# acerbilab/vbmc

Measured on AMD Instinct MI355X. Metric: ELBO+grad evals/sec (Ns=1e4, K=50, D=10, N=400), higher is better.
Workload: dtype f64; 1 GPU; BASELINE configs[2]: D=10 N=400 K=50 Ns=10000/component S=20, R=64 restarts batched per GPU per step, value+gradient, beta=0, no variance; restarts_per_gpu=64, parallelism=one GPU

## Files before the change

### vbmc_amd/csrc/abi_elbo.hip

```cpp
#include <algorithm>
#include <cmath>
#include <mutex>

#include "elbo_kernels.h"
#include "var_kernels.h"
#include "gp_kernels.h"
#include <cstdlib>

extern "C" int vbmc_abi_version(void) { return VBMC_ABI_VERSION; }

static vbmc_status ctx_create_impl(int device, void* stream, vbmc_ctx** out, bool with_aux) {
  if (!out) return VBMC_ERR_INVALID;
  *out = nullptr;
  {
    static std::once_flag hq_once;
    std::call_once(hq_once, [] {
      const char* hq = getenv("VBMC_HW_QUEUES");
      if (!(hq && !strcmp(hq, "0"))) (void)setenv("GPU_MAX_HW_QUEUES", hq && atoi(hq) > 0 ? hq : "8", 0);
    });
  }
  int ndev = 0;
  if (hipGetDeviceCount(&ndev) != hipSuccess || ndev <= 0) return VBMC_ERR_NO_DEVICE;
  if (device < 0 || device >= ndev) return VBMC_ERR_NO_DEVICE;
  hipDeviceProp_t prop;
// ... 362 lines not shown
  if (qs < 1 || qs > 9) return false;
  return fns[qs - 1](kt, grad ? 1 : 0, hv, g.x, g.y, g.z, (void*)st, &ea) == 0;
}
static int entropy_mfma_occupancy(int qs, int kt, int hv, bool grad, const EntArgs& ea) {
  typedef int (*fn_t)(int, int, int, const EntArgs*);
  static const fn_t fns[9] = {vbmc_occupancy_ent_mfma_qs1, vbmc_occupancy_ent_mfma_qs2, vbmc_occupancy_ent_mfma_qs3,
                              vbmc_occupancy_ent_mfma_qs4, vbmc_occupancy_ent_mfma_qs5, vbmc_occupancy_ent_mfma_qs6,
                              vbmc_occupancy_ent_mfma_qs7, vbmc_occupancy_ent_mfma_qs8, vbmc_occupancy_ent_mfma_qs9};
  if (qs < 1 || qs > 9) return -1;
  struct Key { int qs, kt, hv, grad, co, sparse, ldsk; };
  static std::vector<std::pair<Key, int>> cache;
  static std::mutex mu;
  std::lock_guard<std::mutex> lock(mu);
  const Key k{qs, kt, hv, grad ? 1 : 0, ea.lj.rows > 0 ? 1 : 0, ea.cutoff > 0.0 ? 1 : 0, ea.K * (ea.D + ENTP_EXTRA)};
  for (const auto& c : cache)
    if (c.first.qs == k.qs && c.first.kt == k.kt && c.first.hv == k.hv && c.first.grad == k.grad && c.first.co == k.co &&
        c.first.sparse == k.sparse && c.first.ldsk == k.ldsk) return c.second;
  const int nb = fns[qs - 1](kt, grad ? 1 : 0, hv, &ea);
  cache.push_back({k, nb});
  return nb;
}
static bool mfma_entropy_fits(int D, int K, double cutoff, int* qs_out, int* kt_out, int* hv_out) {
  const int qs = (D + 2 + 3) / 4;
  int hv = K <= 64 ? ent_hv_small(qs, K) : (K <= 128 ? ent_hv_mid(qs, K) : (K <= 256 ? 4 : 8));
  if (K > 64 && K <= 128)
    if (const char* f = getenv("VBMC_ENT_HV")) { const int v = atoi(f); if (v == 2 || v == 4) hv = v; }
  if (K > 32 && K <= 64)
    if (const char* f = getenv("VBMC_ENT_HV")) { const int v = atoi(f); if (v == 1 || v == 2) hv = v; }
  int kt = (((K + hv - 1) / hv) + 15) / 16;
  static const bool tail_on = [] { const char* e = getenv("VBMC_ENT_TAIL"); return !(e && !strcmp(e, "0")); }();
  {
    const int Kh = (K + hv - 1) / hv;
    static const int tail_max = [] { const char* e = getenv("VBMC_ENT_TAIL"); return e ? atoi(e) : 2; }();
    const int tl = (Kh % 16 + 3) / 4;
    const int ktf = Kh / 16, rem = Kh % 16;
    const bool tail8_ok = ktf == 1 || (hv == 1 && ktf == 2 && (qs >= 5 || rem <= 6)) || (hv == 1 && ktf == 3 && qs <= 4) ||
                          (hv > 1 && ktf == 2) || (hv > 1 && ktf == 3 && qs >= 5);
    if (tail_on && hv != 8 && Kh > 16 && tl >= 1 && tl <= tail_max && (tl == 1 || (tl == 2 && tail8_ok)) && !(cutoff > 0.0) && !(hv > 1 && ktf < 2)) {
      kt = ktf;
      hv += 16 * tl;
    }
  }
  *qs_out = qs; *kt_out = kt; *hv_out = hv;
  return qs >= 1 && qs <= 9 && K >= 1 && K <= 512 && kt >= 1 && kt <= 4 && !(hv == 2 && kt < 2) && !(hv == 4 && kt < 2) && !(hv == 8 && kt < 3) && !(hv > 16 && kt > 3);
}

#define COPY_KERNEL_MAX_BYTES ((size_t)4 << 20)
__global__ void k_copy_f64(size_t n, const double* __restrict__ src, double* __restrict__ dst) {
  VB_SMALL_PRIO();
  for (size_t i = (size_t)blockIdx.x * blockDim.x + threadIdx.x; i < n; i += (size_t)gridDim.x * blockDim.x) dst[i] = src[i];
}
__global__ void k_copy_rows_f64(int rows, size_t stride, size_t width, const double* __restrict__ src, double* __restrict__ dst) {
  VB_SMALL_PRIO();
  for (int r = blockIdx.y; r < rows; r += gridDim.y)
    for (size_t i = (size_t)blockIdx.x * blockDim.x + threadIdx.x; i < width; i += (size_t)gridDim.x * blockDim.x)
      dst[(size_t)r * stride + i] = src[(size_t)r * stride + i];
}
__global__ void k_pack_sepk(int R, int S, int K, int LJS, int diag_only, const double* __restrict__ lj, const double* __restrict__ J,
                            double* __restrict__ hI, double* __restrict__ hJ) {
  const size_t nI = (size_t)R * S * K, nJ = J ? (size_t)R * S * K * K : 0;
  for (size_t i = (size_t)blockIdx.x * blockDim.x + threadIdx.x; i < nI + nJ; i += (size_t)gridDim.x * blockDim.x) {
    if (i < nI) {
      const int s = (int)(i % S), k = (int)((i / S) % K), r = (int)(i / ((size_t)S * K));
      hI[i] = lj[(((size_t)r * S + s) * K + k) * LJS];
    } else {
      const size_t q = i - nI;
      const int s = (int)(q % S), j = (int)((q / S) % K), k = (int)((q / ((size_t)S * K)) % K), r = (int)(q / ((size_t)S * K * K));
      hJ[q] = (diag_only && j != k) ? 0.0 : J[(((size_t)r * S + s) * K + k) * K + j];
    }
  }
}

static bool copy_by_kernel(size_t bytes) { return bytes <= COPY_KERNEL_MAX_BYTES; }
// ... 1145 lines not shown
  return VBMC_OK;
}

static int limit_T_vargrad() {
  int T = 1;
  while (VAR_FINAL_LDS(1, 1, T + 1) <= 160 * 1024) ++T;
  return T;
}
extern "C" vbmc_status vbmc_get_limits(vbmc_limits* out) {
  if (!out || out->struct_size != sizeof(vbmc_limits)) return VBMC_ERR_INVALID;
  out->max_D = VBMC_LIM_D;
  out->max_K = VBMC_LIM_K;
  out->max_N = trsm_max_n();
  out->max_Na = VBMC_LIM_NA;
  out->max_T_vargrad = limit_T_vargrad();
  out->delta_ok = 1;
  out->meanfun_mask = VBMC_LIM_MEANFUN_MASK;
  return VBMC_OK;
}

extern "C" int vbmc_entropy_plan(int D, int K, int* qs, int* kt, int* hv, int* tail) {
  if (lane_entropy_fits(D, K, 0.0)) {
    if (qs) *qs = 2 * ((D + 1) / 2);
    if (kt) *kt = 2 * ((K + 1) / 2);
    if (hv) *hv = ENT_LANE_WAVES_HOST;
    if (tail) *tail = 0;
    return 2;
  }
  int q = 0, k = 0, h = 0;
  const bool ok = mfma_entropy_fits(D, K, 0.0, &q, &k, &h);
  if (qs) *qs = q;
  if (kt) *kt = k;
  if (hv) *hv = h & 15;
  if (tail) *tail = h >> 4;
  return ok ? 1 : 0;
}

#ifdef VBMC_INSTRUMENT
extern "C" int vbmc_dbg_fin_read(unsigned long long* out) {
  return (int)hipMemcpyFromSymbol(out, HIP_SYMBOL(g_fin_dbg), 64 * sizeof(unsigned long long), 0, hipMemcpyDeviceToHost);
}
#endif

__global__ void k_test_exp(int n, int variant, const double* __restrict__ x, double* __restrict__ y) {
  __shared__ double tab[VB_EXP_TAB_N];
  for (int t = threadIdx.x; t < VB_EXP_TAB_N; t += blockDim.x) tab[t] = c_exp2_tab[t];
  __syncthreads();
  int i = blockIdx.x * blockDim.x + threadIdx.x;
  if (i < n) y[i] = variant == 2 ? vb_exp_tab<1>(x[i], tab) : (variant ? vb_exp_tab<0>(x[i], tab) : vb_exp(x[i]));
}

#include "exp2_tab1k.h"
__global__ void k_test_exp1k(int n, int variant, const double* __restrict__ x, double* __restrict__ y) {
  __shared__ double tab[VB_EXP_TAB1K_N];
  for (int t = threadIdx.x; t < VB_EXP_TAB1K_N; t += blockDim.x) tab[t] = c_exp2_tab1k[t];
  __syncthreads();
  int i = blockIdx.x * blockDim.x + threadIdx.x;
  if (i < n) {
    double ys;
    asm volatile("v_mul_f64 %0, %1, %2" : "=v"(ys) : "v"(x[i]), "v"(VB_EXP_TAB1K_SCALE));
    const bool quad = variant == 3 ? VB_EXP_TAB1K_QUAD : variant == 5;
    y[i] = quad ? vb_exp_tab1k<true>(ys, tab) : vb_exp_tab1k<false>(ys, tab);
  }
}

extern "C" vbmc_status vbmc_test_exp(vbmc_ctx* ctx, int n, int variant, const double* x, double* y) {
  if (!ctx || n <= 0 || !x || !y) return VBMC_ERR_INVALID;
// ... 28 lines not shown
```

### vbmc_amd/csrc/ent_mfma_inst.hip

```cpp
#include "entropy_mfma.h"

#ifndef QS_VALUE
#error "compile with -DQS_VALUE=<1..9>"
#endif
#define CAT2(a, b) a##b
#define CAT(a, b) CAT2(a, b)

template <int KT, int HV, int TL = 0>
static int launch_kt(int mode, int grad, dim3 grid, hipStream_t st, const EntArgs& ea) {
  constexpr int NPV_ = (4 * QS_VALUE + 15) / 16;
  size_t lds = (size_t)ea.K * (ea.D + ENTP_EXTRA) * sizeof(double);
  size_t after = (size_t)VB_EXP_TAB1K_N * sizeof(double);
  if (HV > 1) after += (size_t)(VBMC_ENT_EO(HV) ? 1 : 2) * HV * NPV_ * 4 * WAVE * sizeof(double);
  if (after > lds) lds = after;
  const void* fn = nullptr;
  if constexpr (HV == 1 && QS_VALUE <= 8) {
    if (ea.lj.rows > 0) fn = (const void*)k_entropy_mfma<QS_VALUE, KT, true, false, 1, TL, true>;
  }
  const bool walk = ea.walk_tpw > 0;
  if (walk && !(HV == 1 && QS_VALUE <= 4 && KT <= 3 && grad && !fn && !ea.eps && !(ea.cutoff > 0.0))) return mode != 0 ? -1 : 1;
  if constexpr (HV == 1 && QS_VALUE <= 4 && KT <= 3) {
    if (!fn && grad && !ea.eps && !(ea.cutoff > 0.0))
      fn = walk ? (const void*)k_entropy_mfma<QS_VALUE, KT, true, false, 1, TL, false, false, true> : (const void*)k_entropy_mfma<QS_VALUE, KT, true, false, 1, TL, false, false>;
  }
// ... 1 lines not shown
    if (ea.cutoff > 0.0 && HV == 1 && !TL) {
      if constexpr (HV == 1 && TL == 0)
        fn = grad ? (const void*)k_entropy_mfma<QS_VALUE, KT, true, true, 1> : (const void*)k_entropy_mfma<QS_VALUE, KT, false, true, 1>;
    } else {
      fn = grad ? (const void*)k_entropy_mfma<QS_VALUE, KT, true, false, HV, TL> : (const void*)k_entropy_mfma<QS_VALUE, KT, false, false, HV, TL>;
    }
  }
  if (lds > 64 * 1024) (void)hipFuncSetAttribute(fn, hipFuncAttributeMaxDynamicSharedMemorySize, (int)lds);
  const int threads = (ea.cutoff > 0.0 && HV == 1 && !TL) ? WAVE : WAVE * HV;
  if (mode == 1) {
    int nb = 0;
    if (hipOccupancyMaxActiveBlocksPerMultiprocessor(&nb, fn, threads, lds) != hipSuccess) { (void)hipGetLastError(); return 0; }
    return nb;
  }
  EntArgs arg = ea;
  void* args[] = {(void*)&arg};
  (void)hipLaunchKernel(fn, grid, dim3(threads), args, lds, st);
  return 0;
}

static int dispatch(int mode, int kt, int grad, int hv, dim3 grid, hipStream_t st, const EntArgs* ea) {
  switch (kt + 16 * hv) {
    case 16 + 1: return launch_kt<1, 1>(mode, grad, grid, st, *ea);
    case 16 + 2: return launch_kt<2, 1>(mode, grad, grid, st, *ea);
    case 16 + 3: return launch_kt<3, 1>(mode, grad, grid, st, *ea);
    case 16 + 4: return launch_kt<4, 1>(mode, grad, grid, st, *ea);
    case 272 + 1: return launch_kt<1, 1, 1>(mode, grad, grid, st, *ea);
    case 272 + 2: return launch_kt<2, 1, 1>(mode, grad, grid, st, *ea);
    case 272 + 3: return launch_kt<3, 1, 1>(mode, grad, grid, st, *ea);
    case 288 + 2: return launch_kt<2, 2, 1>(mode, grad, grid, st, *ea);
    case 288 + 3: return launch_kt<3, 2, 1>(mode, grad, grid, st, *ea);
    case 320 + 2: return launch_kt<2, 4, 1>(mode, grad, grid, st, *ea);
    case 320 + 3: return launch_kt<3, 4, 1>(mode, grad, grid, st, *ea);
    case 528 + 1: return launch_kt<1, 1, 2>(mode, grad, grid, st, *ea);
    case 528 + 2: return launch_kt<2, 1, 2>(mode, grad, grid, st, *ea);
    case 528 + 3: return launch_kt<3, 1, 2>(mode, grad, grid, st, *ea);
    case 544 + 2: return launch_kt<2, 2, 2>(mode, grad, grid, st, *ea);
    case 544 + 3: return launch_kt<3, 2, 2>(mode, grad, grid, st, *ea);
    case 576 + 2: return launch_kt<2, 4, 2>(mode, grad, grid, st, *ea);
    case 576 + 3: return launch_kt<3, 4, 2>(mode, grad, grid, st, *ea);
    case 32 + 2: return launch_kt<2, 2>(mode, grad, grid, st, *ea);
    case 32 + 3: return launch_kt<3, 2>(mode, grad, grid, st, *ea);
    case 32 + 4: return launch_kt<4, 2>(mode, grad, grid, st, *ea);
    case 64 + 2: return launch_kt<2, 4>(mode, grad, grid, st, *ea);
    case 64 + 3: return launch_kt<3, 4>(mode, grad, grid, st, *ea);
    case 64 + 4: return launch_kt<4, 4>(mode, grad, grid, st, *ea);
    case 128 + 3: return launch_kt<3, 8>(mode, grad, grid, st, *ea);
    case 128 + 4: return launch_kt<4, 8>(mode, grad, grid, st, *ea);
    default: return mode != 0 ? -1 : 1;
  }
}

extern "C" int CAT(vbmc_launch_ent_mfma_qs, QS_VALUE)(int kt, int grad, int hv, unsigned gx, unsigned gy, unsigned gz, void* stream,
                                                      const EntArgs* ea) {
  return dispatch(0, kt, grad, hv, dim3(gx, gy, gz), (hipStream_t)stream, ea);
}

extern "C" int CAT(vbmc_occupancy_ent_mfma_qs, QS_VALUE)(int kt, int grad, int hv, const EntArgs* ea) {
  return dispatch(1, kt, grad, hv, dim3(1, 1, 1), nullptr, ea);
}

#ifdef VBMC_INSTRUMENT
extern "C" int CAT(vbmc_dbg_ent_read_qs, QS_VALUE)(unsigned long long* out, size_t n) {
  return (int)hipMemcpyFromSymbol(out, HIP_SYMBOL(g_ent_dbg), n * sizeof(unsigned long long), 0, hipMemcpyDeviceToHost);
}
#endif
// ... 1 lines not shown
```

### vbmc_amd/csrc/entropy_mfma.h

```cpp
#pragma once
#include <type_traits>

#include "device_math.h"
#include "elbo_types.h"
#include "exp2_tab1k.h"
#include "logjoint_body.h"

typedef double mf4 __attribute__((ext_vector_type(4)));
struct EntTileAny { static constexpr bool rt = false, val = true; };
struct EntTileFull { static constexpr bool rt = false, val = false; };
struct EntTilePartial { static constexpr bool rt = false, val = true; };
#define VBMC_ENT_SPLIT(KT_, QS_, TL_, HV_) ((HV_) == 1)

#ifdef VBMC_INSTRUMENT
#define VBMC_DBG_WAVES 32768
__device__ unsigned long long g_ent_dbg[6 * VBMC_DBG_WAVES];
#endif

#define VBMC_STAG_FOR(KT_, QS_, TL_) ((KT_) == 1 || (KT_) == 4 || ((KT_) == 2 && (QS_) >= 6) || ((KT_) == 3 && (QS_) <= ((TL_) ? 5 : 8)))



constexpr bool ent_c2_for(int KT, int QS, int TL, int HV) {
  if (HV == 1) {
// ... 7 lines not shown
    if (KT == 3) return !((TL == 1 && (QS == 5 || QS == 6)) || (TL == 2 && QS == 6));
    return true;
  }
  if (KT == 2) return !((TL == 1 && QS >= 6) || (TL == 2 && QS >= 5));
  if (KT == 3) return !(TL == 1 && QS == 7);
  return QS != 5;
}
constexpr bool ent_gp2_for(int KT, int QS, int TL, int HV) { return !(HV == 1 && KT == 1 && TL == 0 && QS <= 3); }

template <int HV>
__device__ __forceinline__ void ent_sync() {
  __builtin_amdgcn_fence(__ATOMIC_RELEASE, "wavefront");
  __builtin_amdgcn_wave_barrier();
  __builtin_amdgcn_fence(__ATOMIC_ACQUIRE, "wavefront");
}
template <int HV>
__device__ __forceinline__ void ent_sync_wg() {
  if (HV == 1) ent_sync<1>();
  else __syncthreads();
}

template <int QS, int KT, bool GRAD, bool SPARSE, int HV = 1, int TL = 0, bool CO = false, bool EM = true, bool WALK = false>
#define VBMC_ENT_EO(HV_) true
#define VBMC_ENT_ONE_WAVE(KT_, QS_, TL_, HV_) \
  (((HV_) == 1 && (KT_) == 4 && (QS_) >= 5) || ((HV_) == 1 && (KT_) == 3 && (QS_) >= 8) || ((HV_) == 4 && (KT_) == 4 && (QS_) >= 6) || \
   ((HV_) == 4 && (KT_) == 3 && (QS_) >= 9))
#define VBMC_ENT_WAVES(KT_, QS_, TL_, HV_) \
  (VBMC_ENT_ONE_WAVE(KT_, QS_, TL_, HV_) ? 1 : ((((KT_) <= 2 && (QS_) <= 4) && !((KT_) == 2 && (TL_) == 2 && (HV_) == 1)) ? 3 : 2))
__device__ __forceinline__ void ent_mfma_segment(const EntArgs& a, const int c, const int j, const int r, const int t0, const int t1,
                                                 const int pdone, const int ptot) {
  static_assert(!CO || (HV == 1 && QS <= 8 && !SPARSE), "the log-joint role exists for single-wave dense kernels at D <= 30");
  static_assert(!WALK || (HV == 1 && !CO), "the walk exists for single-wave workgroups without the log-joint role");
  static_assert(KT <= 4 && (HV == 1 || HV == 2 || HV == 4 || HV == 8), "larger mixtures are split over the waves of a workgroup (HV = 2, 4; round 5: 8, K <= 512)");
  static_assert(TL == 0 || ((TL == 1 || TL == 2) && !SPARSE), "the component tail (one or two values per lane) exists for the dense kernels only");
  constexpr int TLN = TL > 0 ? TL : 1;
  constexpr bool SP = SPARSE;
  constexpr int DP = 4 * QS;
  constexpr int NPV = (4 * QS + 15) / 16;
  constexpr int QL = QS;
  __shared__ double Et[16 * DP];
  constexpr bool GP2 = GRAD && ent_gp2_for(KT, QS, TL, HV);
  __shared__ double RQ_all[HV][GP2 ? 32 : 16];
  __shared__ double BND_all[HV][SPARSE ? KT * 16 * 3 : 1];
  constexpr int YXN = NPV * 4 * WAVE;
  constexpr bool EO = VBMC_ENT_EO(HV);
  constexpr bool YXSB = HV > 1 && EO;
  constexpr bool US = EO;
  constexpr bool VBL = GRAD && HV == 1 && (KT >= 3 || NPV >= 2);
  __shared__ double VBS_all[HV][VBL ? KT * 4 * NPV * WAVE : 1];
  constexpr bool C2 = EO && !SPARSE && ent_c2_for(KT, QS, TL, HV);
#define ENT_CI(kt_, rr_) (16 * (kt_) + 4 * (rr_) + lg)
  __shared__ __attribute__((aligned(16))) double SCP_all[HV][C2 ? KT * 16 * 2 : 2];
  __shared__ double BTL_all[HV][TL ? 4 * TL * DP : 1];
  constexpr bool NML = HV > 1 && EO;
  __shared__ double NMS_all[HV][NML ? KT * 4 * WAVE : 1];
#ifdef VBMC_INSTRUMENT
  const unsigned long long wckE = wall_clock64();
#endif
  int tid_ = threadIdx.x;
  if (WALK) asm volatile("" : "+v"(tid_));
  const int tid = tid_, wv = tid >> 6, hv = HV == 1 ? 0 : wv, lane = tid & 63;
  const int li = lane & 15, lg = lane >> 4;
  int D_ = a.D, K_ = a.K;
  const double *entp_ = a.entp, *vpd_ = a.vpd;
  double* part_ = a.part;
  if (WALK) asm volatile("" : "+s"(D_), "+s"(K_), "+s"(entp_), "+s"(vpd_), "+s"(part_));
  const int D = D_, K = K_;
  double* RQ = RQ_all[wv];
  double* NMS = NMS_all[wv];
  double* BND = BND_all[hv];
  double* VBS = VBS_all[hv];
  double* BTL = BTL_all[hv];
  double* SCP = SCP_all[hv];
  const int Kh = (K + HV - 1) / HV;
  const int kbase = hv * Kh;
  const int Kw = min(K, kbase + Kh) - kbase;
  const int PSg = D + ENTP_EXTRA;
  extern __shared__ double PB[];
  double* const TAB = PB;
  double* const YX = PB + VB_EXP_TAB1K_N;
  constexpr int NTH0 = WAVE * HV;
  constexpr int NTB0 = (VB_EXP_TAB1K_N + NTH0 - 1) / NTH0;
  double tt[NTB0];
#pragma unroll
  for (int u = 0; u < NTB0; ++u) tt[u] = c_exp2_tab1k[min(tid + u * NTH0, VB_EXP_TAB1K_N - 1)];
  const double sigj = vpd_[(size_t)r * VpLayout{D, K}.stride() + VpLayout{D, K}.sigma() + j];
// ... 61 lines not shown
        else if (cc == D) v = h + hj_neg;
        else if (cc == D + 1) v = fma(h, m2, pk[D + 1]) - cKj;
        else v = 0.0;
        SA[kt][q] = ESC * v;
      }
    }
    SC[kt] = ESC * (!kv ? (lg == 1 ? -1.0e6 : 0.0)
                        : (lg == 0 ? h + hj_neg : (lg == 1 ? fma(h, m2, pk[D + 1]) - cKj : 0.0)));
    if (C2 && lg < 2) SCP[(16 * kt + li) * 2 + lg] = 2.0 * SC[kt];
#pragma unroll
    for (int rr = 0; rr < 4; ++rr) {
      const int k2 = ENT_CI(kt, rr);
      const bool kv2 = k2 < Kw;
      const double* p2 = gp + (size_t)(kv2 ? kbase + k2 : 0) * PSg;
      if (GRAD) {
#pragma unroll
        for (int pv = 0; pv < NPV; ++pv) {
          const int col = 16 * pv + li;
          double v = 0.0;
          if (kv2) {
            if (col == 0) v = p2[D + 2];
            else if (col == 1) v = p2[D + 3];
            else if (col < 2 + D) v = p2[D + 3] * (p2[col - 2] - pj[col - 2]);
          }
          if (VBL) VBS[((kt * 4 + rr) * NPV + pv) * WAVE + lane] = v;
          else VB[VBL ? 0 : kt][rr][pv] = v;
        }
      } else {
        WF[kt][rr] = kv2 ? p2[D + 2] : 0.0;
      }
    }
  }

  double tC0[TLN], tC1[TLN], VBt[TLN][NPV], WFt[TLN], Wt[TLN];
#pragma unroll
  for (int u = 0; u < TLN; ++u) {
    tC0[u] = 0.0; tC1[u] = 0.0; WFt[u] = 0.0; Wt[u] = 0.0;
#pragma unroll
    for (int pv = 0; pv < NPV; ++pv) VBt[u][pv] = 0.0;
  }
  if (TL) {
#pragma unroll
    for (int u = 0; u < TLN; ++u) {
      const int tq = 4 * u + lg;
      const int kq = 16 * KT + tq;
      const bool kvq = kq < Kw;
      const double* pq = gp + (size_t)(kvq ? kbase + kq : 0) * PSg;
      const double h = pq[D];
      double m2 = 0.0;
      for (int d = 0; d < D; ++d) { double t = pq[d] - pj[d]; m2 = fma(t, t, m2); }
      tC0[u] = kvq ? ESC * (h + hj_neg) : 0.0;
      tC1[u] = ESC * (kvq ? fma(h, m2, pq[D + 1]) - cKj : -1.0e6);
      for (int d = li; d < DP; d += 16) BTL[tq * DP + d] = (kvq && d < D) ? ESC * (-2.0 * h * (pq[d] - pj[d])) : 0.0;
      if (GRAD) {
#pragma unroll
        for (int pv = 0; pv < NPV; ++pv) {
          const int col = 16 * pv + li;
          double v = 0.0;
          if (kvq) {
            if (col == 0) v = pq[D + 2];
            else if (col == 1) v = pq[D + 3];
            else if (col < 2 + D) v = pq[D + 3] * (pq[col - 2] - pj[col - 2]);
          }
          VBt[u][pv] = v;
        }
      } else {
        WFt[u] = kvq ? pq[D + 2] : 0.0;
      }
    }
  }

  __syncthreads();
  {
#pragma unroll
    for (int u = 0; u < NTB0; ++u) if (VB_EXP_TAB1K_N % NTH0 == 0 || tid + u * NTH0 < VB_EXP_TAB1K_N) TAB[tid + u * NTH0] = tt[u];
  }
  __syncthreads();

#define SAV(kt_, q_) SA[kt_][q_]
  constexpr int VBR = (VBL && NPV == 1 && HV == 1 && KT == 3 && !CO) ? ((EM && QS <= 4) ? (TL == 2 ? 4 : 10) : 12) : 0;
  double VBreg[VBR > 0 ? VBR : 1];
#pragma unroll
  for (int u = 0; u < VBR; ++u) VBreg[u] = VBS[u * WAVE + lane];
#define VBV(kt_, rr_, pv_) (VBL ? (((kt_) * 4 + (rr_)) * NPV + (pv_) < VBR ? VBreg[(((kt_) * 4 + (rr_)) * NPV + (pv_)) < VBR ? (((kt_) * 4 + (rr_)) * NPV + (pv_)) : 0] : VBS[(((kt_) * 4 + (rr_)) * NPV + (pv_)) * WAVE + lane]) : VB[VBL ? 0 : (kt_)][rr_][pv_])
  double accH = 0.0, accG[NPV], accLG[NPV];
  double pm = 1.0;
  int pe = 0, pcnt = 0;
  double Wacc[KT][4];
#pragma unroll
  for (int pv = 0; pv < NPV; ++pv) { accG[pv] = 0.0; accLG[pv] = 0.0; }
#pragma unroll
  for (int kt = 0; kt < KT; ++kt)
#pragma unroll
    for (int rr = 0; rr < 4; ++rr) Wacc[kt][rr] = 0.0;

#ifdef VBMC_INSTRUMENT
  const unsigned long long wck0 = wall_clock64();
#endif
  const int ntile = (a.Mh + 15) >> 4;
  const double sfm0 = lg == 0 ? 1.0 : 0.0, sfm1 = lg == 1 ? 1.0 : 0.0;
  const int emask = (4 * (QS - 1) + lg < D) ? -1 : 0;
  const int emask2 = (QS >= 2 && 4 * (QS - 2) + lg < D) ? -1 : 0;
  const double* epsr = a.eps ? a.eps + (size_t)r * a.eps_stride_r + (size_t)j * a.Mh * D : nullptr;
  constexpr bool EPF = EM && HV == 1 && QS <= 4 && KT <= 3 && !SPARSE;
  double epre[EPF ? QS : 1];
  auto eps_fetch = [&](const int tile) {
#pragma unroll
    for (int u = 0; u < (EPF ? QS : 0); ++u) {
      const int idx = lane + u * WAVE, i = idx / DP, d = idx - i * DP;
      double v = 0.0;
      if (tile < t1 && d < D && tile * 16 + i < a.Mh) v = epsr[(size_t)(tile * 16 + i) * D + d];
      epre[u] = v;
    }
  };
  if (EPF && epsr) eps_fetch(t0);
  if (!epsr && (HV == 1 || hv == 0))
    for (int idx = lane; idx < 16 * DP; idx += WAVE) Et[idx] = 0.0;
  const int evm1 = emask, evm2 = emask2;
  const double c2u1 = (4 * (QS - 1) + lg == D) ? 1.0 : 0.0, c2o1 = (4 * (QS - 1) + lg == D + 1) ? 1.0 : 0.0;
  const double c2u2 = (QS >= 2 && 4 * (QS - 2) + lg == D) ? 1.0 : 0.0;

  auto tile_body = [&](const int tile, auto pkind) __attribute__((always_inline)) {
    using PK = decltype(pkind);
    const int b0 = tile * 16;
    ent_sync_wg<HV>();
    if (HV > 1 && hv != 0) {
    } else if (EPF && epsr) {
#pragma unroll
      for (int u = 0; u < (EPF ? QS : 0); ++u) Et[lane + u * WAVE] = US ? sigj * epre[u] : epre[u];
      eps_fetch(tile + 1);
    } else if (epsr) {
      for (int idx = lane; idx < 16 * DP; idx += WAVE) {
        const int i = idx / DP, d = idx - i * DP;
// ... 77 lines not shown
            e2nd[rr] = fma(pr.x, u2, pr.y) - n[kt][rr];
          }
          if (NML) {
#pragma unroll
            for (int rr = 0; rr < 4; ++rr) NMS[(kt * 4 + rr) * WAVE + lane] = e2nd[rr];
          } else {
            nm[(EO && !NML) ? kt : 0] = e2nd;
          }
        } else
        if (!SP || ((act >> kt) & 1u)) {
          const mf4 cacc = __builtin_amdgcn_mfma_f64_16x16x4f64(SC[kt], sfc, n[kt], 0, 0, 0);
          n[kt] = cacc;
#pragma unroll
          for (int q = 0; q < QL; ++q)
            n[kt] = __builtin_amdgcn_mfma_f64_16x16x4f64(SAV(kt, q), sfl[q], n[kt], 0, 0, 0);
          if (NML) {
            const mf4 e2nd = 2.0 * cacc - n[kt];
#pragma unroll
            for (int rr = 0; rr < 4; ++rr) NMS[(kt * 4 + rr) * WAVE + lane] = e2nd[rr];
          } else {
            nm[(EO && !NML) ? kt : 0] = 2.0 * cacc - n[kt];
          }
        }
      }
    }

    double ntl[TLN], ntm[TLN];
#pragma unroll
    for (int u = 0; u < TLN; ++u) { ntl[u] = 0.0; ntm[u] = 0.0; }
    if (TL) {
#pragma unroll
      for (int u = 0; u < TLN; ++u) {
        double lt = 0.0;
#pragma unroll
        for (int d = 0; d < DP; ++d) lt = fma(BTL[(4 * u + lg) * DP + d], Et[li * DP + d], lt);
        if (!US) lt *= sigj;
        const double ct = fma(tC0[u], u2, tC1[u]);
        ntl[u] = ct + lt;
        ntm[u] = ct - lt;
      }
    }

    auto exps = [&](mf4 (&x)[KT], auto k0c, auto k1c) {
      constexpr int k0 = decltype(k0c)::value, k1 = decltype(k1c)::value;
#pragma unroll
      for (int kt = k0; kt < k1; ++kt) {
        if (kt < KT - 1) {
          if (!SP || ((act >> kt) & 1u)) x[kt] = vb_exp_tab1k4<VB_EXP_TAB1K_QUAD>(x[kt], TAB);
          else x[kt] = (mf4){0.0, 0.0, 0.0, 0.0};
        } else if (SP && !((act >> (KT - 1)) & 1u)) {
          x[KT - 1] = (mf4){0.0, 0.0, 0.0, 0.0};
        } else if (nr_last == 4) {
          x[KT - 1] = vb_exp_tab1k4<VB_EXP_TAB1K_QUAD>(x[KT - 1], TAB);
        } else {
          mf4 t = x[KT - 1];
          x[KT - 1] = (mf4){0.0, 0.0, 0.0, 0.0};
          x[KT - 1][0] = vb_exp_tab1k<VB_EXP_TAB1K_QUAD>(t[0], TAB);
          if (nr_last > 1) x[KT - 1][1] = vb_exp_tab1k<VB_EXP_TAB1K_QUAD>(t[1], TAB);
          if (nr_last > 2) x[KT - 1][2] = vb_exp_tab1k<VB_EXP_TAB1K_QUAD>(t[2], TAB);
        }
      }
    };
    auto texp = [&](double (&t)[TLN]) {
      if (TL) {
#pragma unroll
        for (int u = 0; u < TLN; ++u) t[u] = vb_exp_tab1k<VB_EXP_TAB1K_QUAD>(t[u], TAB);
      }
    };
    auto pvstep = [&](mf4 (&x)[KT], mf4 (&Y)[NPV], int sg, const double (&tn)[TLN]) {
      constexpr bool TWO = NPV == 1 && KT <= 2;
      mf4 Y2s[TWO ? NPV : 1];
      mf4 (&Y2)[TWO ? NPV : 1] = Y2s;
#pragma unroll
      for (int pv = 0; pv < NPV; ++pv) { Y[pv] = (mf4){0.0, 0.0, 0.0, 0.0}; if (TWO) Y2[pv] = (mf4){0.0, 0.0, 0.0, 0.0}; }
#pragma unroll
      for (int kt = 0; kt < KT - 1; ++kt) {
        if (SP && !((act >> kt) & 1u)) continue;
#pragma unroll
        for (int pv = 0; pv < NPV; ++pv) {
          mf4& Yb = TWO ? Y2[TWO ? pv : 0] : Y[pv];
          Y[pv] = __builtin_amdgcn_mfma_f64_16x16x4f64(x[kt][0], VBV(kt, 0, pv), Y[pv], 0, 0, 0);
          Yb = __builtin_amdgcn_mfma_f64_16x16x4f64(x[kt][1], VBV(kt, 1, pv), Yb, 0, 0, 0);
          Y[pv] = __builtin_amdgcn_mfma_f64_16x16x4f64(x[kt][2], VBV(kt, 2, pv), Y[pv], 0, 0, 0);
          Yb = __builtin_amdgcn_mfma_f64_16x16x4f64(x[kt][3], VBV(kt, 3, pv), Yb, 0, 0, 0);
        }
      }
#pragma unroll
      for (int pv = 0; pv < NPV; ++pv) {
        mf4& Yb = TWO ? Y2[TWO ? pv : 0] : Y[pv];
        if (SP && !((act >> (KT - 1)) & 1u)) { if (TWO) Y[pv] += Yb; continue; }
        Y[pv] = __builtin_amdgcn_mfma_f64_16x16x4f64(x[KT - 1][0], VBV(KT - 1, 0, pv), Y[pv], 0, 0, 0);
        if (nr_last > 1) Yb = __builtin_amdgcn_mfma_f64_16x16x4f64(x[KT - 1][1], VBV(KT - 1, 1, pv), Yb, 0, 0, 0);
        if (nr_last > 2) Y[pv] = __builtin_amdgcn_mfma_f64_16x16x4f64(x[KT - 1][2], VBV(KT - 1, 2, pv), Y[pv], 0, 0, 0);
        if (nr_last > 3) Yb = __builtin_amdgcn_mfma_f64_16x16x4f64(x[KT - 1][3], VBV(KT - 1, 3, pv), Yb, 0, 0, 0);
        if (TL) {
#pragma unroll
          for (int u = 0; u < TLN; ++u) Y[pv] = __builtin_amdgcn_mfma_f64_16x16x4f64(tn[u], VBt[u][pv], Y[pv], 0, 0, 0);
        }
        if (TWO) Y[pv] += Yb;
      }
      if (HV > 1) {
        if (YXSB && sg == 1) __syncthreads();
#pragma unroll
        for (int pv = 0; pv < NPV; ++pv)
#pragma unroll
          for (int rr = 0; rr < 4; ++rr) YX[((YXSB ? 0 : sg) * HV + hv) * YXN + (pv * 4 + rr) * WAVE + lane] = Y[pv][rr];
        __syncthreads();
#pragma unroll
        for (int pv = 0; pv < NPV; ++pv)
#pragma unroll
          for (int rr = 0; rr < 4; ++rr) {
            double t = YX[((YXSB ? 0 : sg) * HV + 0) * YXN + (pv * 4 + rr) * WAVE + lane];
#pragma unroll
            for (int w = 1; w < HV; ++w) t += YX[((YXSB ? 0 : sg) * HV + w) * YXN + (pv * 4 + rr) * WAVE + lane];
            Y[pv][rr] = t;
          }
      }
    };
    auto put_q = [&](mf4 (&Y)[NPV]) {
      if (GP2 ? li < 2 : li == 0) {
#pragma unroll
        for (int rr = 0; rr < 4; ++rr) RQ[(GP2 ? 16 * li : 0) + lg + 4 * rr] = Y[0][rr];
      }
      ent_sync<HV>();
    };
    double arq = 0.0;
    constexpr bool TQ = GP2 && US && NPV == 1 && HV == 1 && EO && KT == 3 && QS <= 3 && !CO && !EM && VBMC_STAG_FOR(KT, QS, TL);
    double tq[TQ ? 4 : 1];
    auto get_rq = [&]() -> double {
      double qs_ = RQ[li];
      double rqs = vb_rcp(qs_);
      if (partial) {
        qs_ = svalid ? qs_ : 1.0;
        rqs = svalid ? rqs : 0.0;
      }
      if (GP2) arq = RQ[GP2 ? 16 + li : 0] * rqs;
      pm *= __builtin_amdgcn_frexp_mant(qs_);
      pe += __builtin_amdgcn_frexp_exp(qs_);
      accH += shift;
      return rqs;
    };
    auto wacc = [&](mf4 (&x)[KT], double rqs, const double (&tn)[TLN]) {
      if (TL) {
#pragma unroll
        for (int u = 0; u < TLN; ++u) Wt[u] = fma(tn[u], rqs, Wt[u]);
      }
#pragma unroll
      for (int kt = 0; kt < KT; ++kt) {
        if (SP && !((act >> kt) & 1u)) continue;
#pragma unroll
        for (int rr = 0; rr < 4; ++rr) Wacc[kt][rr] = fma(x[kt][rr], rqs, Wacc[kt][rr]);
      }
    };
    auto put_rq = [&](double rqs) {
      ent_sync<HV>();
      if (lg == 0) { RQ[li] = rqs; if (GP2) RQ[GP2 ? 16 + li : 0] = arq; }
      ent_sync<HV>();
    };
    auto gradpieces = [&](mf4 (&Y)[NPV], double ssig, auto sgc) {
      constexpr int SG = decltype(sgc)::value;
      if constexpr (GP2) {
#pragma unroll
        for (int rr = 0; rr < 4; ++rr) {
          const int i = lg + 4 * rr;
          const double rq = RQ[i], ar = RQ[GP2 ? 16 + i : 0];
#pragma unroll
          for (int pv = 0; pv < NPV; ++pv) {
            if (HV > 1 && (pv % HV) != hv) continue;
            const int d = min(max(16 * pv + li - 2, 0), DP - 1);
            double tv;
            if (TQ) { if (SG >= 0) tq[TQ ? rr : 0] = Et[i * DP + d]; tv = tq[TQ ? rr : 0]; }
            else tv = Et[i * DP + d];
            const double t = (US && SG > 0) ? tv : ((US && SG < 0) ? -tv : ssig * tv);
            const double gd = fma(t, ar, -(Y[pv][rr] * rq));
            accG[pv] += gd;
            accLG[pv] = fma(t, gd, accLG[pv]);
          }
        }
// ... 11 lines not shown
          if (HV > 1 && (pv % HV) != hv) continue;
          const int d = 16 * pv + li - 2;
          if (d >= 0 && d < D) {
            const double t = (US && SG > 0) ? Et[i * DP + d] : ((US && SG < 0) ? -Et[i * DP + d] : ssig * Et[i * DP + d]);
            const double gd = (t * Av - Y[pv][rr]) * rq;
            accG[pv] += gd;
            accLG[pv] = fma(t, gd, accLG[pv]);
          }
        }
      }
      ent_sync<HV>();
    };
    auto fold = [&]() {
      if (++pcnt == 256) {
        pe += __builtin_amdgcn_frexp_exp(pm);
        pm = __builtin_amdgcn_frexp_mant(pm);
        pcnt = 0;
      }
    };
    using I0 = std::integral_constant<int, 0>;
    using IH = std::integral_constant<int, (KT + 1) / 2>;
    using IK = std::integral_constant<int, KT>;

    if constexpr (EO && GRAD && HV == 1 && VBMC_STAG_FOR(KT, QS, TL)) {
      mf4 Y[NPV];
      exps(n, I0{}, IK{});
      texp(ntl);
      pvstep(n, Y, 0, ntl);
      put_q(Y);
      exps(nm, I0{}, IH{});
      const double rqs = get_rq();
      put_rq(rqs);
      exps(nm, IH{}, IK{});
      texp(ntm);
      wacc(n, rqs, ntl);
      gradpieces(Y, sigj, std::integral_constant<int, 1>{});
      fold();
      pvstep(nm, Y, 1, ntm);
      put_q(Y);
      const double rqs2 = get_rq();
      wacc(nm, rqs2, ntm);
      put_rq(rqs2);
      gradpieces(Y, -sigj, std::integral_constant<int, -1>{});
      fold();
    } else {
      int sg = 0;
      double ssig = US ? 1.0 : sigj;
#pragma unroll 1
      for (;;) {
        if (!EO) {
          double sf[QS];
#pragma unroll
          for (int q = 0; q < QS; ++q) {
            const int cc = 4 * q + lg;
            constexpr bool EVREG = KT <= 3 && QS <= 7;
            sf[q] = (cc < D) ? ssig * (EVREG ? ev[q] : Et[li * DP + 4 * q + lg]) : ((cc == D) ? u2 : ((cc == D + 1) ? 1.0 : 0.0));
          }
#pragma unroll
          for (int kt = 0; kt < KT; ++kt) {
            n[kt] = (mf4){0.0, 0.0, 0.0, 0.0};
#pragma unroll
            for (int q = 0; q < QS; ++q) n[kt] = __builtin_amdgcn_mfma_f64_16x16x4f64(SA[kt][q], sf[q], n[kt], 0, 0, 0);
          }
        }
        exps(n, I0{}, IK{});
        texp(ntl);
        if (GRAD) {
          mf4 Y[NPV];
          pvstep(n, Y, sg, ntl);
          put_q(Y);
          const double rqs = get_rq();
          wacc(n, rqs, ntl);
          put_rq(rqs);
          gradpieces(Y, ssig, std::integral_constant<int, 0>{});
        } else {
          double qp = 0.0;
#pragma unroll
          for (int kt = 0; kt < KT; ++kt)
#pragma unroll
            for (int rr = 0; rr < 4; ++rr) qp = fma(WF[kt][rr], n[kt][rr], qp);
          if (TL) {
#pragma unroll
            for (int u = 0; u < TLN; ++u) qp = fma(WFt[u], ntl[u], qp);
          }
          qp += __shfl_xor(qp, 16, 64);
          qp += __shfl_xor(qp, 32, 64);
          if (HV > 1) {
            if (YXSB && sg == 1) __syncthreads();
            YX[((YXSB ? 0 : sg) * HV + hv) * YXN + lane] = qp;
            __syncthreads();
            qp = YX[((YXSB ? 0 : sg) * HV + 0) * YXN + lane];
#pragma unroll
            for (int w = 1; w < HV; ++w) qp += YX[((YXSB ? 0 : sg) * HV + w) * YXN + lane];
          }
          double qs_ = qp;
          if (partial) qs_ = svalid ? qp : 1.0;
          pm *= __builtin_amdgcn_frexp_mant(qs_);
          pe += __builtin_amdgcn_frexp_exp(qs_);
          accH += shift;
        }
        fold();
        if (sg) break;
        sg = 1;
        ssig = US ? -1.0 : -sigj;
        if (EO) {
#pragma unroll
          for (int kt = 0; kt < KT; ++kt) {
            if (NML) {
#pragma unroll
              for (int rr = 0; rr < 4; ++rr) n[kt][rr] = NMS[(kt * 4 + rr) * WAVE + lane];
            } else {
              n[kt] = nm[(EO && !NML) ? kt : 0];
            }
          }
        }
#pragma unroll
        for (int u = 0; u < TLN; ++u) ntl[u] = ntm[u];
      }
    }
  };
  if constexpr (VBMC_ENT_SPLIT(KT, QS, TL, HV)) {
    const int tf = min(t1, a.Mh >> 4);
    constexpr bool PRIO = CO ? QS <= 4 : VBMC_ENT_WAVES(KT, QS, TL, HV) > 1;
    const bool pr = PRIO && a.prio != 0;
    const int q1 = pr ? t0 + (ptot + 3) / 4 - pdone : -1, q2 = pr ? t0 + (ptot + 1) / 2 - pdone : -1, q3 = pr ? t0 + (3 * ptot + 3) / 4 - pdone : -1;
    if (pr && pdone == 0) __builtin_amdgcn_s_setprio(3);
    for (int tile = t0; tile < tf; ++tile) {
      if (tile == q1) __builtin_amdgcn_s_setprio(2);
      if (tile == q2) __builtin_amdgcn_s_setprio(1);
      if (tile == q3) __builtin_amdgcn_s_setprio(0);
      tile_body(tile, EntTileFull{});
    }
    if (tf < t1) tile_body(tf, EntTilePartial{});
  } else {
    for (int tile = t0; tile < t1; ++tile) tile_body(tile, EntTileAny{});
  }
#ifdef VBMC_INSTRUMENT
  const unsigned long long wck1 = wall_clock64();
#endif
  if (WALK) accH += vb_log_pos(pm, &pe) + 0.693147180559945309417 * (double)pe;
  else accH += log(pm) + 0.693147180559945309417 * (double)pe;
  if (lg != 0) accH = 0.0;

  double* o = part_ + (((size_t)r * K + j) * a.C + c) * a.ncol;
  accH = wave_sum(accH);
  if (lane == 0 && hv == 0) o[0] = accH;
  if (GRAD) {
    double sgsum = 0.0;
#pragma unroll
    for (int pv = 0; pv < NPV; ++pv) {
      double g = accG[pv], lgd = accLG[pv] / sigj;
      g += __shfl_xor(g, 16, 64); g += __shfl_xor(g, 32, 64);
      lgd += __shfl_xor(lgd, 16, 64); lgd += __shfl_xor(lgd, 32, 64);
      const int d = 16 * pv + li - 2;
      const bool dv = d >= 0 && d < D;
      const bool mine = HV == 1 || (pv % HV) == hv;
      if (dv && lg == 0 && mine) { o[1 + d] = g; o[2 + D + d] = lgd; }
      sgsum += (dv && lg == 0 && mine) ? lgd : 0.0;
    }
    sgsum = wave_sum(sgsum);
    if (HV > 1) {
      __syncthreads();
      if (lane == 0) YX[hv * YXN] = sgsum;
      __syncthreads();
      sgsum = YX[0];
#pragma unroll
      for (int w = 1; w < HV; ++w) sgsum += YX[w * YXN];
    }
    if (lane == 0 && hv == 0) o[1 + D] = sgsum;
#pragma unroll
    for (int kt = 0; kt < KT; ++kt)
#pragma unroll
      for (int rr = 0; rr < 4; ++rr) {
        double wv = Wacc[kt][rr];
        wv += __shfl_xor(wv, 1, 64); wv += __shfl_xor(wv, 2, 64);
        wv += __shfl_xor(wv, 4, 64); wv += __shfl_xor(wv, 8, 64);
        const int k = ENT_CI(kt, rr);
        if (li == 0 && k < Kw) o[2 + 2 * D + kbase + k] = wv;
      }
    if (TL) {
#pragma unroll
      for (int u = 0; u < TLN; ++u) {
        double wv = Wt[u];
        wv += __shfl_xor(wv, 1, 64); wv += __shfl_xor(wv, 2, 64);
        wv += __shfl_xor(wv, 4, 64); wv += __shfl_xor(wv, 8, 64);
        const int k = 16 * KT + 4 * u + lg;
        if (li == 0 && k < Kw) o[2 + 2 * D + kbase + k] = wv;
      }
    }
  }
#ifdef VBMC_INSTRUMENT
  if (lane == 0) {
    const size_t w = ((size_t)r * K + j) * a.C + c;
    if (w < VBMC_DBG_WAVES) {
      g_ent_dbg[6 * w + 0] = wckE; g_ent_dbg[6 * w + 1] = wck0; g_ent_dbg[6 * w + 2] = wck1; g_ent_dbg[6 * w + 3] = wall_clock64();
      g_ent_dbg[6 * w + 4] = __builtin_amdgcn_s_getreg(63492);
      g_ent_dbg[6 * w + 5] = __builtin_amdgcn_s_getreg(63508);
    }
  }
#endif
#undef VBV
#undef SAV
#undef ENT_CI
}

template <int QS, int KT, bool GRAD, bool SPARSE, int HV = 1, int TL = 0, bool CO = false, bool EM = true, bool WALK = false>
__global__ void __launch_bounds__(WAVE * HV, CO ? (QS <= 4 ? 2 : 1) : VBMC_ENT_WAVES(KT, QS, TL, HV)) k_entropy_mfma(EntArgs a) {
  const int ntile = (a.Mh + 15) >> 4;
  constexpr bool walk = WALK;
  int c = (int)blockIdx.x, j = CO ? (int)blockIdx.y - a.lj.rows : (int)blockIdx.y, r = (int)blockIdx.z;
  int tlo = ((int)blockIdx.x + a.c0) * a.tiles_per_chunk, thi = min(tlo + a.tiles_per_chunk, ntile), pdone = 0, rem = 0;
  if (!WALK && a.co_c2 > 0 && c >= a.co_c1) {
    tlo = a.co_c1 * a.tiles_per_chunk + (c - a.co_c1) * a.co_tpc2;
    thi = min(tlo + a.co_tpc2, ntile);
  }
  if (CO) {
    if ((int)blockIdx.y < a.lj.rows) {
      extern __shared__ double PB[];
      lj_co_role<4 * QS>(a.lj, a.vpd, PB);
      const int e = (int)(blockIdx.y * gridDim.x + blockIdx.x);
// ... 32 lines not shown
```

Before: 29910 evals/s.

## Add sign-split component tail variant for single-wave three-tile entropy kernels

Adds a new tail mode (TL=3) for the MFMA entropy kernel, used when the leftover components after three full k-tiles number at most two. The +sigma and -sigma antithetic halves share one tail register slot instead of two, with lane groups 0-1 holding the plus sign and 2-3 the minus sign. This drops the second tail exp evaluation and the ntm bookkeeping. The cost is an extra cross-lane shuffle when reducing the tail weights and more template instantiations. The D=10, K=50 case (Kh=50, three full tiles, remainder 2) falls into this path.

```diff
diff --git a/vbmc_amd/csrc/abi_elbo.hip b/vbmc_amd/csrc/abi_elbo.hip
--- a/vbmc_amd/csrc/abi_elbo.hip
+++ b/vbmc_amd/csrc/abi_elbo.hip
@@ -418,13 +418,15 @@
   {
     const int Kh = (K + hv - 1) / hv;
     static const int tail_max = [] { const char* e = getenv("VBMC_ENT_TAIL"); return e ? atoi(e) : 2; }();
+    static const bool tail_sp = [] { const char* e = getenv("VBMC_ENT_TAIL_SPLIT"); return !(e && !strcmp(e, "0")); }();
     const int tl = (Kh % 16 + 3) / 4;
     const int ktf = Kh / 16, rem = Kh % 16;
     const bool tail8_ok = ktf == 1 || (hv == 1 && ktf == 2 && (qs >= 5 || rem <= 6)) || (hv == 1 && ktf == 3 && qs <= 4) ||
                           (hv > 1 && ktf == 2) || (hv > 1 && ktf == 3 && qs >= 5);
     if (tail_on && hv != 8 && Kh > 16 && tl >= 1 && tl <= tail_max && (tl == 1 || (tl == 2 && tail8_ok)) && !(cutoff > 0.0) && !(hv > 1 && ktf < 2)) {
       kt = ktf;
-      hv += 16 * tl;
+      const bool tsp = tl == 1 && hv == 1 && ktf == 3 && rem <= 2 && qs <= 4 && tail_sp;
+      hv += 16 * (tsp ? 3 : tl);
     }
   }
   *qs_out = qs; *kt_out = kt; *hv_out = hv;
@@ -1636,7 +1638,7 @@
   if (qs) *qs = q;
   if (kt) *kt = k;
   if (hv) *hv = h & 15;
-  if (tail) *tail = h >> 4;
+  if (tail) *tail = (h >> 4) == 3 ? 1 : h >> 4;
   return ok ? 1 : 0;
 }
 
diff --git a/vbmc_amd/csrc/ent_mfma_inst.hip b/vbmc_amd/csrc/ent_mfma_inst.hip
--- a/vbmc_amd/csrc/ent_mfma_inst.hip
+++ b/vbmc_amd/csrc/ent_mfma_inst.hip
@@ -57,6 +57,9 @@
     case 288 + 3: return launch_kt<3, 2, 1>(mode, grad, grid, st, *ea);
     case 320 + 2: return launch_kt<2, 4, 1>(mode, grad, grid, st, *ea);
     case 320 + 3: return launch_kt<3, 4, 1>(mode, grad, grid, st, *ea);
+    case 784 + 3:
+      if constexpr (QS_VALUE <= 4) return launch_kt<3, 1, 3>(mode, grad, grid, st, *ea);
+      else return mode != 0 ? -1 : 1;
     case 528 + 1: return launch_kt<1, 1, 2>(mode, grad, grid, st, *ea);
     case 528 + 2: return launch_kt<2, 1, 2>(mode, grad, grid, st, *ea);
     case 528 + 3: return launch_kt<3, 1, 2>(mode, grad, grid, st, *ea);
diff --git a/vbmc_amd/csrc/entropy_mfma.h b/vbmc_amd/csrc/entropy_mfma.h
--- a/vbmc_amd/csrc/entropy_mfma.h
+++ b/vbmc_amd/csrc/entropy_mfma.h
@@ -63,8 +63,11 @@
   static_assert(!CO || (HV == 1 && QS <= 8 && !SPARSE), "the log-joint role exists for single-wave dense kernels at D <= 30");
   static_assert(!WALK || (HV == 1 && !CO), "the walk exists for single-wave workgroups without the log-joint role");
   static_assert(KT <= 4 && (HV == 1 || HV == 2 || HV == 4 || HV == 8), "larger mixtures are split over the waves of a workgroup (HV = 2, 4; round 5: 8, K <= 512)");
-  static_assert(TL == 0 || ((TL == 1 || TL == 2) && !SPARSE), "the component tail (one or two values per lane) exists for the dense kernels only");
-  constexpr int TLN = TL > 0 ? TL : 1;
+  static_assert(TL == 0 || ((TL == 1 || TL == 2 || TL == 3) && !SPARSE), "the component tail (one or two values per lane) exists for the dense kernels only");
+  static_assert(TL != 3 || (HV == 1 && KT == 3 && QS <= 4), "the sign-split tail is built for single-wave kernels of three k-tiles at D <= 14");
+  constexpr bool TSP = TL == 3;
+  constexpr int TLN = TL == 0 ? 1 : (TSP ? 1 : TL);
+  constexpr int TLW = TSP ? 2 : TLN;
   constexpr bool SP = SPARSE;
   constexpr int DP = 4 * QS;
   constexpr int NPV = (4 * QS + 15) / 16;
@@ -82,7 +85,7 @@
   constexpr bool C2 = EO && !SPARSE && ent_c2_for(KT, QS, TL, HV);
 #define ENT_CI(kt_, rr_) (16 * (kt_) + 4 * (rr_) + lg)
   __shared__ __attribute__((aligned(16))) double SCP_all[HV][C2 ? KT * 16 * 2 : 2];
-  __shared__ double BTL_all[HV][TL ? 4 * TL * DP : 1];
+  __shared__ double BTL_all[HV][TL ? 4 * TLN * DP : 1];
   constexpr bool NML = HV > 1 && EO;
   __shared__ double NMS_all[HV][NML ? KT * 4 * WAVE : 1];
 #ifdef VBMC_INSTRUMENT
@@ -210,17 +213,19 @@
     }
   }
 
-  double tC0[TLN], tC1[TLN], VBt[TLN][NPV], WFt[TLN], Wt[TLN];
-#pragma unroll
-  for (int u = 0; u < TLN; ++u) {
-    tC0[u] = 0.0; tC1[u] = 0.0; WFt[u] = 0.0; Wt[u] = 0.0;
+  double tC0[TLN], tC1[TLN], VBt[TLW][NPV], WFt[TLN], Wt[TLW];
+#pragma unroll
+  for (int u = 0; u < TLN; ++u) { tC0[u] = 0.0; tC1[u] = 0.0; WFt[u] = 0.0; }
+#pragma unroll
+  for (int u = 0; u < TLW; ++u) {
+    Wt[u] = 0.0;
 #pragma unroll
     for (int pv = 0; pv < NPV; ++pv) VBt[u][pv] = 0.0;
   }
   if (TL) {
 #pragma unroll
     for (int u = 0; u < TLN; ++u) {
-      const int tq = 4 * u + lg;
+      const int tq = TSP ? (lg & 1) : 4 * u + lg;
       const int kq = 16 * KT + tq;
       const bool kvq = kq < Kw;
       const double* pq = gp + (size_t)(kvq ? kbase + kq : 0) * PSg;
@@ -229,7 +234,8 @@
       for (int d = 0; d < D; ++d) { double t = pq[d] - pj[d]; m2 = fma(t, t, m2); }
       tC0[u] = kvq ? ESC * (h + hj_neg) : 0.0;
       tC1[u] = ESC * (kvq ? fma(h, m2, pq[D + 1]) - cKj : -1.0e6);
-      for (int d = li; d < DP; d += 16) BTL[tq * DP + d] = (kvq && d < D) ? ESC * (-2.0 * h * (pq[d] - pj[d])) : 0.0;
+      if (!TSP || lg < 2)
+        for (int d = li; d < DP; d += 16) BTL[tq * DP + d] = (kvq && d < D) ? ESC * (-2.0 * h * (pq[d] - pj[d])) : 0.0;
       if (GRAD) {
 #pragma unroll
         for (int pv = 0; pv < NPV; ++pv) {
@@ -240,7 +246,12 @@
             else if (col == 1) v = pq[D + 3];
             else if (col < 2 + D) v = pq[D + 3] * (pq[col - 2] - pj[col - 2]);
           }
-          VBt[u][pv] = v;
+          if (TSP) {
+            VBt[0][pv] = lg < 2 ? v : 0.0;
+            VBt[TLW - 1][pv] = lg < 2 ? 0.0 : v;
+          } else {
+            VBt[u][pv] = v;
+          }
         }
       } else {
         WFt[u] = kvq ? pq[D + 2] : 0.0;
@@ -277,6 +288,7 @@
 #endif
   const int ntile = (a.Mh + 15) >> 4;
   const double sfm0 = lg == 0 ? 1.0 : 0.0, sfm1 = lg == 1 ? 1.0 : 0.0;
+  const double tsg = lg < 2 ? 1.0 : -1.0;
   const int emask = (4 * (QS - 1) + lg < D) ? -1 : 0;
   const int emask2 = (QS >= 2 && 4 * (QS - 2) + lg < D) ? -1 : 0;
   const double* epsr = a.eps ? a.eps + (size_t)r * a.eps_stride_r + (size_t)j * a.Mh * D : nullptr;
@@ -420,12 +432,17 @@
 #pragma unroll
       for (int u = 0; u < TLN; ++u) {
         double lt = 0.0;
-#pragma unroll
-        for (int d = 0; d < DP; ++d) lt = fma(BTL[(4 * u + lg) * DP + d], Et[li * DP + d], lt);
+        const int tr = TSP ? (lg & 1) : 4 * u + lg;
+#pragma unroll
+        for (int d = 0; d < DP; ++d) lt = fma(BTL[tr * DP + d], Et[li * DP + d], lt);
         if (!US) lt *= sigj;
         const double ct = fma(tC0[u], u2, tC1[u]);
-        ntl[u] = ct + lt;
-        ntm[u] = ct - lt;
+        if (TSP) {
+          ntl[u] = fma(lt, tsg, ct);
+        } else {
+          ntl[u] = ct + lt;
+          ntm[u] = ct - lt;
+        }
       }
     }
 
@@ -483,7 +500,7 @@
         if (nr_last > 3) Yb = __builtin_amdgcn_mfma_f64_16x16x4f64(x[KT - 1][3], VBV(KT - 1, 3, pv), Yb, 0, 0, 0);
         if (TL) {
 #pragma unroll
-          for (int u = 0; u < TLN; ++u) Y[pv] = __builtin_amdgcn_mfma_f64_16x16x4f64(tn[u], VBt[u][pv], Y[pv], 0, 0, 0);
+          for (int u = 0; u < TLN; ++u) Y[pv] = __builtin_amdgcn_mfma_f64_16x16x4f64(tn[u], VBt[TSP ? (TSP && sg ? TLW - 1 : 0) : u][pv], Y[pv], 0, 0, 0);
         }
         if (TWO) Y[pv] += Yb;
       }
@@ -528,10 +545,13 @@
       accH += shift;
       return rqs;
     };
-    auto wacc = [&](mf4 (&x)[KT], double rqs, const double (&tn)[TLN]) {
+    auto wacc = [&](mf4 (&x)[KT], double rqs, const double (&tn)[TLN], int sg) {
       if (TL) {
 #pragma unroll
-        for (int u = 0; u < TLN; ++u) Wt[u] = fma(tn[u], rqs, Wt[u]);
+        for (int u = 0; u < TLN; ++u) {
+          double& w = Wt[TSP ? (TSP && sg ? TLW - 1 : 0) : u];
+          w = fma(tn[u], rqs, w);
+        }
       }
 #pragma unroll
       for (int kt = 0; kt < KT; ++kt) {
@@ -609,14 +629,14 @@
       const double rqs = get_rq();
       put_rq(rqs);
       exps(nm, IH{}, IK{});
-      texp(ntm);
-      wacc(n, rqs, ntl);
+      if (!TSP) texp(ntm);
+      wacc(n, rqs, ntl, 0);
       gradpieces(Y, sigj, std::integral_constant<int, 1>{});
       fold();
-      pvstep(nm, Y, 1, ntm);
+      pvstep(nm, Y, 1, TSP ? ntl : ntm);
       put_q(Y);
       const double rqs2 = get_rq();
-      wacc(nm, rqs2, ntm);
+      wacc(nm, rqs2, TSP ? ntl : ntm, 1);
       put_rq(rqs2);
       gradpieces(Y, -sigj, std::integral_constant<int, -1>{});
       fold();
@@ -641,13 +661,13 @@
           }
         }
         exps(n, I0{}, IK{});
-        texp(ntl);
+        if (!TSP || sg == 0) texp(ntl);
         if (GRAD) {
           mf4 Y[NPV];
           pvstep(n, Y, sg, ntl);
           put_q(Y);
           const double rqs = get_rq();
-          wacc(n, rqs, ntl);
+          wacc(n, rqs, ntl, sg);
           put_rq(rqs);
           gradpieces(Y, ssig, std::integral_constant<int, 0>{});
         } else {
@@ -658,7 +678,7 @@
             for (int rr = 0; rr < 4; ++rr) qp = fma(WF[kt][rr], n[kt][rr], qp);
           if (TL) {
 #pragma unroll
-            for (int u = 0; u < TLN; ++u) qp = fma(WFt[u], ntl[u], qp);
+            for (int u = 0; u < TLN; ++u) qp = fma((!TSP || (lg >> 1) == sg) ? WFt[u] : 0.0, ntl[u], qp);
           }
           qp += __shfl_xor(qp, 16, 64);
           qp += __shfl_xor(qp, 32, 64);
@@ -691,8 +711,10 @@
             }
           }
         }
-#pragma unroll
-        for (int u = 0; u < TLN; ++u) ntl[u] = ntm[u];
+        if (!TSP) {
+#pragma unroll
+          for (int u = 0; u < TLN; ++u) ntl[u] = ntm[u];
+        }
       }
     }
   };
@@ -758,11 +780,12 @@
     if (TL) {
 #pragma unroll
       for (int u = 0; u < TLN; ++u) {
-        double wv = Wt[u];
+        double wv = TSP ? (lg < 2 ? Wt[0] : Wt[TLW - 1]) : Wt[u];
         wv += __shfl_xor(wv, 1, 64); wv += __shfl_xor(wv, 2, 64);
         wv += __shfl_xor(wv, 4, 64); wv += __shfl_xor(wv, 8, 64);
+        if (TSP) wv += __shfl_xor(wv, 32, 64);
         const int k = 16 * KT + 4 * u + lg;
-        if (li == 0 && k < Kw) o[2 + 2 * D + kbase + k] = wv;
+        if (li == 0 && k < Kw && (!TSP || lg < 2)) o[2 + 2 * D + kbase + k] = wv;
       }
     }
   }
```

After: 30070 evals/s, median of 6. No clear change (+0.6%).
